# StefanHeng/ECG-Representation-Learning

Measured on AMD Instinct MI355X. Metric: 12-lead ECG records/sec pre-train step, ViT-Base bf16 @ 1/2/4/8 MI355X, higher is better.
Workload: dtype bf16

## Files before the change

### __graft_entry__.py

```python
import os
import subprocess
import sys

ROOT = os.path.dirname(os.path.abspath(__file__))
CSRC = os.path.join(ROOT, 'ecg-representation-learning_amd', 'csrc')
if ROOT not in sys.path:
    sys.path.insert(0, ROOT)


def build() -> None:
    env = dict(os.environ)
    env.setdefault('HIPCC', '/opt/rocm/bin/hipcc')
    jobs = f'-j{min(8, os.cpu_count() or 1)}'
    subprocess.run(['make', '-C', CSRC, jobs, 'all'], check=True, env=env)
    import ecg_representation_learning_amd as E
    lib = E.hip.lib()
    assert lib.ecgvit_abi_version() == E.hip.ABI_VERSION
    for name in E.hip.SIGNATURES:
        getattr(lib, name)
    r = subprocess.run(['make', '-C', CSRC, jobs, 'tools'], env=env)
    if r.returncode != 0:
        print('WARNING: the tools library did not build (the product library did); tests that need tools/toolslib.py will fail', file=sys.stderr)


def smoke() -> None:
    import torch
    import ecg_representation_learning_amd as E
    from oracle import vit_oracle as O
    assert torch.cuda.is_available(), 'smoke() needs cuda:0'
    torch.manual_seed(77)
    conf = E.EcgVitConfig(max_signal_length=1000, patch_size=20, hidden_size=128, num_hidden_layers=2,
                          num_attention_heads=2, intermediate_size=256, hidden_dropout_prob=0., attention_probs_dropout_prob=0.)
    x, y = O.synthetic_batch(4, length=1000, seed=77)
    ref = O.OracleEcgVit(config=conf)
    ref.train()
    out_ref = ref(sample_values=x, labels=y)
    out_ref.loss.backward()
    for dtype, tol in ((torch.float32, 1e-4), (torch.bfloat16, 3e-2)):
        m = E.EcgVit(config=conf, compute_dtype=dtype)
        m.load_state_dict(ref.state_dict())
        m.cuda().train()
        out = m(sample_values=x.cuda(), labels=y.cuda())
        out.loss.backward()
        rel = abs(float(out.loss) - float(out_ref.loss)) / abs(float(out_ref.loss))
        g = m.vit.mlp_head[1].weight.grad.cpu()
        g_ref = ref.vit.mlp_head[1].weight.grad
        grel = float((g - g_ref).norm() / g_ref.norm())
        print(f'smoke[{dtype}]: loss {float(out.loss):.6f} vs oracle {float(out_ref.loss):.6f} (rel {rel:.2e}); head-grad rel {grel:.2e}')
        assert rel < tol and grel < 30 * tol, (dtype, rel, grel)
        step = E.HipTrainStep(m, dict(n_step=10), sync_nonfinite=True)
        loss, _ = step.step(x.cuda(), y.cuda())
# ... 78 lines not shown
```

### ecg-representation-learning_amd/engine.py

```python
import math
from collections import OrderedDict

import os

import torch

from . import hip
from .hip import lib, run, ptr, stream, GEMM_NT, GEMM_NN, GEMM_TN
from .hip import EPI_BIAS, EPI_GELU, EPI_GELU_BWD, EPI_RESIDUAL, EPI_DROPOUT, EPI_COLSUM, EPI_GELU_GRAD_AUX, EPI_MUL_AUX

LN_EPS = 1e-5


def _align(n, a=8):
    return (n + a - 1) // a * a


def _numel(shape):
    n = 1
    for v in shape:
        n *= v
    return n


class ParamLayout:

    def __init__(self, named_shapes):
        self.entries = OrderedDict()
        off = 0
        for name, shape in named_shapes:
            n = _numel(shape)
            self.entries[name] = (off, tuple(shape), n)
            off = _align(off + n, 16)
        self.total = off

    def view(self, flat, name):
# ... 346 lines not shown
        if d > hip.ROW_MAX_D:
            raise ValueError(f'HIP LayerNorm kernels cover hidden_size <= {hip.ROW_MAX_D}')
        if h == 1:
            raise NotImplementedError('heads == 1 (vit_pytorch drops to_out) is not covered by the HIP path')
        if dtype == torch.bfloat16:
            if self.dh not in (64, 128):
                raise ValueError(f'bf16 fused attention needs head dim 64 or 128 (got {self.dh}); use dtype=torch.float32')
            if self.N > hip.ATTN_MAX_N:
                raise ValueError(f'bf16 fused attention covers <= {hip.ATTN_MAX_N} tokens (got {self.N}); use dtype=torch.float32')
            for nm, pv in (('hidden_dropout_prob', self.p_hidden), ('attention_probs_dropout_prob (the embedding dropout: reference ecg_vit.py:113)', self.p_emb)):
                if 0.0 < pv < 1.0 / 512:
                    raise ValueError(f'the bf16 path applies dropout in steps of 1/256: {nm}={pv} would round to no dropout; use 0, a value '
                                     f'>= 1/512, or compute_dtype=torch.float32 (exact p)')
        self.fp8 = bool(fp8_linear)
        if self.fp8:
            if dtype != torch.bfloat16:
                raise ValueError('fp8_linear needs the bf16 engine (compute_dtype=torch.bfloat16)')
            if d % 128 or f % 128:
                raise ValueError(f'fp8_linear needs hidden_size and intermediate_size to be multiples of 128 (got d={d}, f={f})')
        self.fp8_drop_dead_bf16 = self.fp8 and d % 256 == 0 and f % 256 == 0
        if saved_ffn_e4m3 and dtype != torch.bfloat16:
            raise ValueError('saved_ffn_e4m3 needs the bf16 engine (the f32 parity path keeps the f32 pre-activation)')
        self.aux8 = dtype == torch.bfloat16 if saved_ffn_e4m3 is None else bool(saved_ffn_e4m3)
        self.B = None
        self._alloc_key = None
        self._pool, self._pool_B = None, 0
        self.T = self.N
        self.act = None
        self.P32 = self.G32 = self.W = None
        self._ws = {}
        self.saved = None
        self.input_transform = None
        self.on_grads_ready = None
        self._tpw = 0

    def _set_width(self, width):
        if width == self.L:
            return
        if not 0 < width <= self.L_max or width % self.P:
            raise ValueError(f'a batch of {width} samples per record: must be a positive multiple of patch_size={self.P} '
                             f'and at most max_signal_length={self.L_max}')
        self.L, self.n = width, width // self.P
        self.N = self.n + 1

    def _gemm(self, *a, **kw):
        kw.setdefault('tiles_per_workgroup', self._tpw)
        hip.gemm(*a, **kw)

    def bind(self, pflat, gflat, wlow=None, wlow_t=None):
        lay = self.layout
        self.P32 = {k: lay.view(pflat, k) for k in lay.entries}
        self.G32 = {k: lay.view(gflat, k) for k in lay.entries}
        self.WT = {}
        if self.dtype == torch.bfloat16:
            assert wlow is not None and wlow.dtype == torch.bfloat16
            self.W = {k: lay.view(wlow, k) for k in lay.entries}
            if wlow_t is not None:
                for k in self.transposed_weight_names():
                    off, shape = lay.entries[k][0], lay.entries[k][1]
                    self.WT[k] = wlow_t[off:off + shape[0] * shape[1]].view(shape[1], shape[0])
        else:
            self.W = self.P32
        self.device = pflat.device
        if self.fp8:
            assert wlow_t is not None, 'fp8_linear runs the input gradients against the transposed weight shadows'
            names = self.transposed_weight_names()
# ... 177 lines not shown

    def _act_spec(self, B, masked, m, rows=None, N=None, mrows=None):
        T = self.dtype
        f32, u8 = torch.float32, torch.uint8
        if N is None:
            N = self.n if masked else self.N
        M, Mp = B * N, B * (N if masked else N - 1)
        if rows is not None:
            M, Mp = rows, rows - (0 if masked else B)
        d, f, h = self.d, self.f, self.h
        sp = OrderedDict()
        sp.update(patches=((Mp, self.CP), T), tok=((Mp, d), T), x0=((M, d), T))
        for i in range(self.Ly):
            l = dict(mean1=((M,), f32), rstd1=((M,), f32), xn1=((M, d), T), qkv=((M, 3 * d), T), attn=((M, d), T), x1=((M, d), T),
                     mean2=((M,), f32), rstd2=((M,), f32), xn2=((M, d), T), hpre=((M, f), u8 if self._aux8(M) else T), hact=((M, f), T), x2=((M, d), T))
            if T == torch.float32:
                l['probs'] = ((B * h * N * N,), T)
            else:
                l['lse'] = ((B * h * N,), f32)
            if self.fp8 and M >= 2048:
                l.update(xn1_8=((M * d,), u8), attn_8=((M * d,), u8), xn2_8=((M * d,), u8), hact_8=((M * f,), u8))
            for k, v in l.items():
                sp[f'L{i}.{k}'] = v
        sp.update(logits=((B, self.K), f32), xhat=((B, d), f32), hrstd=((B,), f32), loss_elem=((B, self.K), f32), loss_mean=((1,), f32),
                  dlogits=((B, self.K), f32))
        sp.update(dxa=((M, d), T), dxb=((M, d), T), dxn=((M, d), T), dqkv=((M, 3 * d), T), dattn=((M, d), T), dh=((M, f), T),
                  dtok=((Mp, d), T), dxm=((M, d), T))
        if T == torch.float32:
            sp.update(pd=((B * h * N * N,), T), dp=((B * h * N * N,), T))
        if T == torch.bfloat16 and not masked:
            sp.update({f'cls_{k}': ((B, d), T) for k in ('attn', 'x1', 'xn2', 'x2', 'dx', 'dy', 'dxn', 'dx1', 'dxm', 'dattn', 'dq')})
            sp.update(cls_hpre=((B, f), T), cls_hact=((B, f), T), cls_dh=((B, f), T), cls_lse=((B * h,), f32), cls_mean2=((B,), f32),
                      cls_rstd2=((B,), f32))
        l = lib()
        ws = max(l.ecgvit_layernorm_bwd_workspace(M, d), l.ecgvit_colsum_workspace(M, max(f, 3 * d)), 8 * ((M + 255) // 256) * f, 4096)
        if T == torch.bfloat16:
            for (mm, nn) in ((d, f), (f, d), (d, d), (3 * d, d), (d, self.CP)):
                ws = max(ws, hip.gemm_workspace_bytes(GEMM_TN, T, mm, nn, M))
        if masked:
            Rm = B * m if mrows is None else mrows
            sp.update(flag=((Mp,), u8), rows=((Rm, d), T), pred=((Rm, self.CP), T), target=((Rm, self.CP), T),
                      dpred=((Rm, self.CP), T), drows=((Rm, d), T), dmasked=((Mp, d), T), mloss=((1,), f32), l1part=((1024,), f32))
        sp['ws'] = ((ws,), u8)
        if self.fp8:
            sp['q8'] = ((M * max(f, 3 * d),), u8)
            sp['q8b'] = ((M * f,), u8)
        return sp

    def _ln_fwd(self, x, g, b, y, mean, rstd, rows, q8_site=None, y8=None):
        d = self.d
        if (self.fp8 and q8_site is not None and q8_site in self._f8_seen and rows >= 2048 and d % 256 == 0
                and d // 64 in (4, 8, 12, 16, 24, 32)):
            run.ecgvit_layernorm_fwd_q8(ptr(x), ptr(g), ptr(b), None if (y8 is not None and self._only8(rows)) else ptr(y), ptr(mean), ptr(rstd), rows, d, LN_EPS,
                                        ptr(y8 if y8 is not None else self.act['q8']),
                                        ptr(self.f8_scale[q8_site:q8_site + 1]), ptr(self.f8_amax[q8_site:q8_site + 1]), stream())
            return True
        run.ecgvit_layernorm_fwd(ptr(x), ptr(g), ptr(b), ptr(y), ptr(mean), ptr(rstd), rows, d, LN_EPS,
                                 hip.code(self.dtype), stream())
        return False

    def _ln_bwd(self, dy, x, g, mean, rstd, dres, dx, dg, db, rows):
        run.ecgvit_layernorm_bwd(ptr(dy), ptr(x), ptr(g), ptr(mean), ptr(rstd), ptr(dres), ptr(dx), ptr(dg), ptr(db),
                                 ptr(self.act['ws']), rows, self.d, hip.code(self.dtype), stream())

    def _ln_bwd_fused(self, dy, x, g, mean, rstd, dres, dx, dg, db, rows, dxm, dcolsum, p, seed, q8_site=None):
        d = self.d
# ... 146 lines not shown
            if (self.fp8 and self._pass_rows(B) >= 2048 and site in self._f8_seen and dh == 64 and 128 < N <= 512
                    and N * 3 * d * 2 < 2 ** 31):
                run.ecgvit_attention_bwd_q8(ptr(L['qkv']), ptr(L['attn']), ptr(a['dattn']), ptr(L['lse']), ptr(a['dqkv']), B, N, h, dh, self.scale,
                                            ph, seed, ptr(a['q8']), ptr(self.f8_scale[site:site + 1]), ptr(self.f8_amax[site:site + 1]), st)
                return True
            run.ecgvit_attention_bwd(ptr(L['qkv']), ptr(L['attn']), ptr(a['dattn']), ptr(L['lse']), ptr(a['dqkv']), B, N, h, dh, self.scale, ph,
                                     seed, hip.BF16, st)
        else:
            self._attn_bwd_f32(L, B, ph, seed)
        return False

    def _attention_cls_fwd(self, L, B, ph, seed):
        a, st = self.act, stream()
        h, dh, N = self.h, self.dh, self.T
        ntok = self.saved.get('ntok')
        if ntok is not None:
            run.ecgvit_attention_varlen_cls_fwd(ptr(L['qkv']), ptr(a['cls_attn']), ptr(a['cls_lse']), ptr(ntok), B, N, h, dh, self.scale, ph, seed,
                                                st)
        else:
            run.ecgvit_attention_cls_fwd(ptr(L['qkv']), ptr(a['cls_attn']), ptr(a['cls_lse']), B, N, h, dh, self.scale, ph, seed,
                                         hip.code(self.dtype), st)

    def _attention_cls_bwd(self, L, B, ph, seed):
        a, st = self.act, stream()
        h, dh, N = self.h, self.dh, self.T
        ntok = self.saved.get('ntok')
        if ntok is not None:
            run.ecgvit_attention_varlen_cls_bwd(ptr(L['qkv']), ptr(a['cls_attn']), ptr(a['cls_dattn']), ptr(a['cls_lse']), ptr(a['dqkv']),
                                                ptr(a['cls_dq']), ptr(ntok), B, N, h, dh, self.scale, ph, seed, st)
        else:
            run.ecgvit_attention_cls_bwd(ptr(L['qkv']), ptr(a['cls_attn']), ptr(a['cls_dattn']), ptr(a['cls_lse']), ptr(a['dqkv']), ptr(a['cls_dq']),
                                         B, N, h, dh, self.scale, ph, seed, hip.code(self.dtype), st)

    def _cls_block_fwd(self, L, X, B, ph, s0, lp):
        a, W, P = self.act, self.W, self.P32
        d, f, N = self.d, self.f, self.T
        M = B * N
        self._ln_fwd(X, P[lp + '0.norm.weight'], P[lp + '0.norm.bias'], L['xn1'], L['mean1'], L['rstd1'], M)
        wqkv = W[lp + '0.fn.to_qkv.weight']
        self._gemm(GEMM_NT, L['xn1'], wqkv, L['qkv'], M, 2 * d, d, d, d, 3 * d, b_off=d * d, c_off=d)
        self._gemm(GEMM_NT, L['xn1'], wqkv, L['qkv'], B, d, d, N * d, d, N * 3 * d)
        self._attention_cls_fwd(L, B, ph, s0 + 1)
        drop = EPI_DROPOUT if ph > 0 else 0
        self._gemm(GEMM_NT, a['cls_attn'], W[lp + '0.fn.to_out.0.weight'], a['cls_x1'], B, d, d, d, d, d, epilogue=EPI_BIAS | EPI_RESIDUAL | drop,
                   bias=P[lp + '0.fn.to_out.0.bias'], residual=X, ldr=N * d, dropout_p=ph, seed=s0 + 2, mask_row_pitch=N)
        self._ln_fwd(a['cls_x1'], P[lp + '1.norm.weight'], P[lp + '1.norm.bias'], a['cls_xn2'], a['cls_mean2'], a['cls_rstd2'], B)
        self._gemm(GEMM_NT, a['cls_xn2'], W[lp + '1.fn.net.0.weight'], a['cls_hact'], B, f, d, d, d, f,
                   epilogue=EPI_BIAS | EPI_GELU | EPI_GELU_GRAD_AUX | drop, bias=P[lp + '1.fn.net.0.bias'], aux=a['cls_hpre'], ldaux=f,
                   dropout_p=ph, seed=s0 + 3, mask_row_pitch=N)
        self._gemm(GEMM_NT, a['cls_hact'], W[lp + '1.fn.net.3.weight'], a['cls_x2'], B, d, f, f, f, d, epilogue=EPI_BIAS | EPI_RESIDUAL | drop,
                   bias=P[lp + '1.fn.net.3.bias'], residual=a['cls_x1'], ldr=d, dropout_p=ph, seed=s0 + 4, mask_row_pitch=N)
        return a['cls_x2']

    def forward(self, x, labels=None, weight=None, training=True, seed=0, want_mean=True, cls_only_last=False, lengths=None):
        return self._head_loss(self._trunk_pass(x, labels, weight, training, seed, cls_only_last, lengths), want_mean)

    def _head_loss(self, X, want_mean):
        a, sv, T = self.act, self.saved, hip.code(self.dtype)
        st = stream()
        B, d, rg, labels = sv['B'], self.d, sv['ragged'], sv['labels']
        pre = 'vit.'
        sv['head_pitch'] = 1 if (sv['cls_only_last'] or rg is not None) else self.N
        if rg is not None:
            run.ecgvit_gather_rows(ptr(X), ptr(rg.tok_off), ptr(a['cls_x2']), 1, rg.M, B, d, d, d, T, st)
            X = a['cls_x2']
        run.ecgvit_head_fwd(ptr(X), sv['head_pitch'], ptr(self.P32[pre + 'mlp_head.0.weight']), ptr(self.P32[pre + 'mlp_head.0.bias']),
                            ptr(self.P32[pre + 'mlp_head.1.weight']), ptr(self.P32[pre + 'mlp_head.1.bias']),
                            ptr(a['logits']), ptr(a['xhat']), ptr(a['hrstd']), B, d, self.K, LN_EPS, T, st)
        if labels is None:
            return a['logits'], None, None
        run.ecgvit_bce_fwd(ptr(a['logits']), ptr(labels), ptr(sv['weight']), ptr(a['loss_elem']),
                           ptr(a['loss_mean']) if want_mean else None, B * self.K, st)
        return a['logits'], a['loss_elem'], (a['loss_mean'] if want_mean else None)

    def _trunk_pass(self, x, labels, weight, training, seed, cls_only_last, lengths):
# ... 444 lines not shown
        i = self.Ly - 1
        L = a['layers'][i]
        lp = f'vit.transformer.layers.{i}.'
        s0 = seed + 100 * (i + 1)
        Xin = a['x0'] if i == 0 else a['layers'][i - 1]['x2']
        dY = dXc
        if ph > 0:
            run.ecgvit_dropout_apply_rows(ptr(dXc), ptr(a['cls_dy']), B, d, N, ph, s0 + 4, T, st)
            dY = a['cls_dy']
        self._colsum(dY, d, G[lp + '1.fn.net.3.bias'], B, d)
        if self._wants(lp + '1.fn.net.3.weight'):
            self._gemm(GEMM_TN, dY, a['cls_hact'], G[lp + '1.fn.net.3.weight'], d, f, B, d, f, f, workspace=ws)
        b = self._stage(i, 0)
        if not self._reach(b):
            return None, None
        self._gemm(GEMM_NN, dY, W[lp + '1.fn.net.3.weight'], a['cls_dh'], B, f, d, d, f, f, epilogue=EPI_MUL_AUX | EPI_COLSUM, aux=a['cls_hpre'],
                   ldaux=f, workspace=ws, colsum_out=G[lp + '1.fn.net.0.bias'])
        if self._wants(lp + '1.fn.net.0.weight'):
            self._gemm(GEMM_TN, a['cls_dh'], a['cls_xn2'], G[lp + '1.fn.net.0.weight'], f, d, B, f, d, d, workspace=ws)
        if not self._reach(b + 1):
            return None, None
        self._gemm(GEMM_NN, a['cls_dh'], W[lp + '1.fn.net.0.weight'], a['cls_dxn'], B, d, f, f, d, d)
        if not self._reach(b + 2):
            return None, None
        run.ecgvit_layernorm_bwd_fused_rowpitch(ptr(a['cls_dxn']), ptr(a['cls_x1']), ptr(P[lp + '1.norm.weight']), ptr(a['cls_mean2']),
                                                ptr(a['cls_rstd2']), ptr(dXc), ptr(a['cls_dx1']), ptr(G[lp + '1.norm.weight']),
                                                ptr(G[lp + '1.norm.bias']), ptr(ws), B, d, ptr(a['cls_dxm']), ptr(G[lp + '0.fn.to_out.0.bias']),
                                                ph, s0 + 2, N, T, st)
        dY = a['cls_dxm'] if ph > 0 else a['cls_dx1']
        if self._wants(lp + '0.fn.to_out.0.weight'):
            self._gemm(GEMM_TN, dY, a['cls_attn'], G[lp + '0.fn.to_out.0.weight'], d, d, B, d, d, d, workspace=ws)
        if not self._reach(b + 3):
            return None, None
        self._gemm(GEMM_NN, dY, W[lp + '0.fn.to_out.0.weight'], a['cls_dattn'], B, d, d, d, d, d)
        if not self._reach(b + 4):
            return None, None
        self._attention_cls_bwd(L, B, ph, s0 + 1)
        name = lp + '0.fn.to_qkv.weight'
        if self._wants(name):
            self._gemm(GEMM_TN, a['dqkv'], L['xn1'], G[name], 2 * d, d, M, 3 * d, d, d, workspace=ws, a_off=d, c_off=d * d)
            self._gemm(GEMM_TN, a['cls_dq'], L['xn1'], G[name], d, d, B, d, N * d, d, workspace=ws)
        if not self._reach(b + 5):
            return None, None
        wt = self.WT.get(name)
        if wt is not None and M >= 2048:
            self._gemm(GEMM_NT, a['dqkv'], wt, a['dxn'], M, d, 2 * d, 3 * d, 3 * d, d, a_off=d, b_off=d)
        else:
            self._gemm(GEMM_NN, a['dqkv'], W[name], a['dxn'], M, d, 2 * d, 3 * d, d, d, a_off=d, b_off=d * d)
        self._gemm(GEMM_NN, a['cls_dq'], W[name], a['dxn'], B, d, d, d, d, N * d, epilogue=hip.EPI_ACCUM)
        if not self._reach(b + 6):
            return None, None
        dres.zero_()
        run.ecgvit_scatter_rows(ptr(a['cls_dx1']), ptr(self._cls_rows(B)), ptr(dres), B, N, 1, d, d, d, T, st)
        if i > 0:
            lq = f'vit.transformer.layers.{i - 1}.'
            self._ln_bwd_fused(a['dxn'], Xin, P[lp + '0.norm.weight'], L['mean1'], L['rstd1'], dres, out, G[lp + '0.norm.weight'],
                               G[lp + '0.norm.bias'], M, a['dxm'], G[lq + '1.fn.net.3.bias'], ph, seed + 100 * i + 4)
        else:
            self._ln_bwd(a['dxn'], Xin, P[lp + '0.norm.weight'], L['mean1'], L['rstd1'], dres, out, G[lp + '0.norm.weight'], G[lp + '0.norm.bias'], M)
        self._ready(f'layer{i}')
        return out, dres

    def _cls_rows(self, B):
        t = getattr(self, '_cls_idx', None)
        if t is None or t.numel() < B or t.device != self.device:
            t = self._cls_idx = torch.zeros(max(B, 1), dtype=torch.int32, device=self.device)
        return t[:B]

    def _attn_bwd_f32(self, L, B, ph, seed):
        d, h, dh, N = self.d, self.h, self.dh, self.T
        a = self.act
        qkv, P, dqkv, dO, dP = L['qkv'], L['probs'], a['dqkv'], a['dattn'], a['dp']
        sq, so, sp = (N * 3 * d, dh), (N * d, dh), (h * N * N, N * N)
        Pd = P
        if ph > 0:
            Pd = a['pd']
            self._drop_apply_f32(P, Pd, B * h * N * N, ph, seed)
        self._gemm(GEMM_TN, Pd, dO, dqkv, N, dh, N, N, d, 3 * d, batch=(B, h), strideA=sp, strideB=so, strideC=sq, c_off=2 * d)
        self._gemm(GEMM_NT, dO, qkv, dP, N, N, dh, d, 3 * d, N, batch=(B, h), strideA=so, strideB=sq, strideC=sp, b_off=2 * d)
        if ph > 0:
# ... 61 lines not shown
```

### ecg-representation-learning_amd/hip.py

```python
import ctypes
import os
from ctypes import c_int, c_int32, c_int64, c_uint64, c_float, c_double, c_void_p, c_char_p, POINTER, Structure, byref

import torch

_PKG_DIR = os.path.dirname(os.path.abspath(__file__))
LIB_PATH = os.path.join(_PKG_DIR, 'libecgvit_hip.so')

ABI_VERSION = 6
F32, BF16, FP8_E4M3, BF8_E5M2 = 0, 1, 2, 3
GEMM_NT, GEMM_NN, GEMM_TN = 0, 1, 2
EPI_BIAS, EPI_GELU, EPI_GELU_BWD, EPI_RESIDUAL, EPI_ACCUM, EPI_DROPOUT, EPI_COLSUM = 1, 2, 4, 8, 16, 32, 64
EPI_GELU_GRAD_AUX, EPI_MUL_AUX, EPI_QUANT_OUT, EPI_NO_OUT, EPI_AUX8 = 128, 256, 512, 1024, 2048

ACC_INIT, ACC_ADD, ACC_FOLD = 0, 1, 2
KERNEL_NONE, KERNEL_GEMM_F32, KERNEL_GEMM_BF16, KERNEL_GEMM_NT, KERNEL_GEMM_WGRAD = 0, 1, 2, 3, 4
POOL_CLS, POOL_MEAN = 0, 1
ATTN_MAX_N, ROW_MAX_D = 2048, 2048
FIT_TARGETS, FIT_BINS = 16, 256
DENOISE_MAX_LEN, DENOISE_MAX_LEN_TILED = 32768, 33554432
DENOISE_MAX_TAPS = 9
DENOISE_MAX_POINTS, DENOISE_MAX_ROBUST_ITERS = 1024, 10
DENOISE_NLM_RUN, DENOISE_NLM_MAX_THREADS = 15, 512
DENOISE_LOESS_LDS = 4096
DENOISE_MAX_TILES = 65535
RESAMPLE_MAX_LEN, RESAMPLE_MAX_CHIRP = 33554432, 16777216
RESAMPLE_MAX_GENERIC, RESAMPLE_MAX_GRID_Y = 65536, 65535
TOK_MAX_CLUSTERS, TOK_MAX_LOCAL_TRIALS = 65536, 16
TOK_SEED_SPAN, TOK_DBSCAN_TILE = 1024, 256

_ERR = {1: 'ECGVIT_EINVAL (unsupported shape / argument)', 2: 'ECGVIT_ELAUNCH (HIP launch failure)'}


class HipLibraryMissing(ImportError):
    pass


class GemmDesc(Structure):
    _fields_ = [
        ('layout', c_int32), ('dtype', c_int32), ('out_dtype', c_int32), ('epilogue', c_int32),
        ('M', c_int32), ('N', c_int32), ('K', c_int32), ('batch1', c_int32), ('batch2', c_int32),
        ('A', c_void_p), ('lda', c_int64), ('strideA1', c_int64), ('strideA2', c_int64),
        ('B', c_void_p), ('ldb', c_int64), ('strideB1', c_int64), ('strideB2', c_int64),
        ('C', c_void_p), ('ldc', c_int64), ('strideC1', c_int64), ('strideC2', c_int64),
        ('bias', c_void_p), ('residual', c_void_p), ('ldr', c_int64), ('aux', c_void_p), ('ldaux', c_int64),
        ('alpha', c_float), ('dropout_p', c_float), ('dropout_seed', c_uint64),
        ('workspace', c_void_p), ('workspace_bytes', c_int64), ('colsum_out', c_void_p), ('tiles_per_workgroup', c_int32),
        ('q8_out', c_void_p), ('ldq8', c_int64), ('q8_scale', c_void_p), ('q8_amax', c_void_p), ('q8_format', c_int32),
        ('scale_a', c_void_p), ('scale_b', c_void_p),
    ]

# ... 80 lines not shown
    'ecgvit_fit_select': (c_int, [_P, _P, _I, _I, _I, _P]),
    'ecgvit_tok_assign': (c_int, [_P, _P, _L, _P, _P, _P, _L, _I, _I, _L, _I, _I, _P, _I, _P, _P, _P, _P, _P, _P]),
    'ecgvit_tok_workspace': (c_int64, [_I, _I]),
    'ecgvit_tok_update': (c_int, [_P, _P, _L, _P, _P, _P, _L, _I, _I, _L, _I, _I, _P, _P, _I, _P, _P, _I, _P]),
    'ecgvit_tok_seed_workspace': (c_int64, [_I, _L, _I, _I, _I]),
    'ecgvit_tok_seed': (c_int, [_P, _P, _L, _P, _P, _P, _L, _I, _I, _L, _I, _I, _I, _I, _L, _P, _P, _P, _P, _P, _I, _P]),
    'ecgvit_tok_decode': (c_int, [_P, _P, _L, _P, _P, _P, _L, _I, _I, _L, _I, _P, _P, _P, _I, _P]),
    'ecgvit_tok_segments': (c_int, [_P, _P, _L, _P, _P, _P, _L, _I, _I, _L, _I, _I, _P, _P, _P, _P]),
    'ecgvit_tok_dbscan_tile': (c_int, []),
    'ecgvit_tok_dbscan_rows': (c_int, [_I]),
    'ecgvit_tok_dbscan_count': (c_int, [_P, _I, _I, _F, _I, _I, _P, _P]),
    'ecgvit_tok_dbscan_link': (c_int, [_P, _I, _I, _F, _I, _I, _P, _P]),
    'ecgvit_tok_dbscan_flatten': (c_int, [_P, _I, _P, _P]),
    'ecgvit_tok_dbscan_border': (c_int, [_P, _I, _P, _P, _I, _I, _F, _I, _I, _P, _P]),
    'ecgvit_denoise_workspace': (c_int64, [_I, _I, _I]),
    'ecgvit_filtfilt': (c_int, [_P, _P, _P, _L, _P, _I, _I, _I, _I, POINTER(c_double), POINTER(c_double), POINTER(c_double), _I, _P, _P]),
    'ecgvit_nlm_sigma': (c_int, [_P, _P, _L, _P, _I, _I, _I, _P, _P, _P]),
    'ecgvit_nlm_denoise': (c_int, [_P, _P, _P, _L, _P, _I, _I, _I, _P, _D, _I, _I, _P]),
    'ecgvit_rloess': (c_int, [_P, _P, _P, _L, _P, _I, _I, _I, _I, _I, _D, _I, _I, _I, _P, _P]),
    'ecgvit_denoise_workspace_long': (c_int64, [_I, _I, _I]),
    'ecgvit_filtfilt_long': (c_int, [_P, _P, _P, _L, _P, _I, _I, _I, _I, POINTER(c_double), POINTER(c_double), POINTER(c_double), _I, _P, _P]),
    'ecgvit_nlm_sigma_long': (c_int, [_P, _P, _L, _P, _I, _I, _I, _P, _P, _P]),
    'ecgvit_nlm_denoise_tiled': (c_int, [_P, _P, _P, _L, _P, _I, _I, _I, _P, _D, _I, _I, _I, _P]),
    'ecgvit_rloess_tiled': (c_int, [_P, _P, _P, _L, _P, _I, _I, _I, _I, _I, _D, _I, _I, _I, _P, _I, _P]),
    'ecgvit_resample_plan': (c_int, [_I, POINTER(c_int), _I]),
    'ecgvit_resample_workspace': (c_int64, [_I, _I, _I, _I]),
    'ecgvit_resample': (c_int, [_P, _P, _P, _L, _P, _L, _I, _I, _I, _I, _P, _P, _P, _P]),
    'ecgvit_resample_chirp_length': (c_int, [_I]),
    'ecgvit_resample_chirp_workspace': (c_int64, [_I, _I, _I, _I, _I, _I]),
    'ecgvit_resample_chirp_filter': (c_int, [_P, _I, _I, _P, _P, _P, _P]),
    'ecgvit_resample_chirp': (c_int, [_P, _P, _P, _L, _P, _L, _I, _I, _I, _I, _P, _P, _P, _P, _P, _P, _P, _P]),
}

_lib = None


def use_library(path):
    global LIB_PATH
    if _lib is not None:
        raise RuntimeError('use_library() must come before the first ecgvit call of the process')
    if not os.path.exists(path):
        raise HipLibraryMissing(f'{path} not found')
    LIB_PATH = os.path.abspath(path)


def lib():
    global _lib
    if _lib is None:
        if not os.path.exists(LIB_PATH):
            raise HipLibraryMissing(
                f'{LIB_PATH} not found: build it with `python -c "import __graft_entry__ as g; g.build()"` '
                f'(or `make -C {os.path.join(_PKG_DIR, "csrc")}`). There is no CPU / eager fallback.')
        l = ctypes.CDLL(LIB_PATH)
        for name, (res, args) in SIGNATURES.items():
            fn = getattr(l, name)
            fn.restype, fn.argtypes = res, args
        _lib = l
    return _lib


def check(rc, what):
    if rc != 0:
        raise RuntimeError(f'{what}: {_ERR.get(rc, rc)}')


_QUERIES = frozenset(('ecgvit_abi_version', 'ecgvit_gemm_kernel', 'ecgvit_resample_plan', 'ecgvit_resample_chirp_length', 'ecgvit_tok_dbscan_tile',
                      'ecgvit_tok_dbscan_rows'))


class _Run:

    def __getattr__(self, name):
        if name not in SIGNATURES or name in _QUERIES or SIGNATURES[name][0] is not c_int:
            raise AttributeError(f'{name}: not an entry point that returns a status (queries go through lib())')
        fns = vars(lib())

        def call(*args):
            rc = fns[name](*args)
            if rc:
                raise RuntimeError(f'{name}: {_ERR.get(rc, rc)}')
        call.__name__ = name
        setattr(self, name, call)
        return call


run = _Run()


def ptr(t):
    return None if t is None else t.data_ptr()


def stream():
    return torch.cuda.current_stream().cuda_stream


def code(dtype):
    if dtype == torch.float32:
        return F32
    if dtype == torch.bfloat16:
        return BF16
    raise ValueError(f'unsupported activation dtype {dtype}')


def _need_cuda(*ts):
    for t in ts:
# ... 49 lines not shown
```

### include/ecgvit_hip.h

```cpp
#ifndef ECGVIT_HIP_H
#define ECGVIT_HIP_H

#include <stdint.h>

#ifdef __cplusplus
extern "C" {
#endif

#define ECGVIT_OK 0
#define ECGVIT_EINVAL 1
#define ECGVIT_ELAUNCH 2

#define ECGVIT_F32 0
#define ECGVIT_BF16 1
#define ECGVIT_FP8_E4M3 2
#define ECGVIT_BF8_E5M2 3

const char *ecgvit_version(void);
int ecgvit_abi_version(void);

#define ECGVIT_GEMM_NT 0
#define ECGVIT_GEMM_NN 1
#define ECGVIT_GEMM_TN 2

// ... 83 lines not shown
                               void *dxm, float *dcolsum, float dropout_p, uint64_t seed, int dtype, void *stream);

int ecgvit_layernorm_bwd_fused_rowpitch(const void *dy, const void *x, const float *gamma, const float *mean, const float *rstd,
                                        const void *dres, void *dx, float *dgamma, float *dbeta, void *partial, int64_t rows, int d,
                                        void *dxm, float *dcolsum, float dropout_p, uint64_t seed, int mask_row_pitch, int dtype, void *stream);

int ecgvit_layernorm_bwd_fused_q8(const void *dy, const void *x, const float *gamma, const float *mean, const float *rstd,
                                  const void *dres, void *dx, float *dgamma, float *dbeta, void *partial, int64_t rows, int d,
                                  void *dxm, float *dcolsum, float dropout_p, uint64_t seed, void *g8, const float *q8_scale,
                                  float *q8_amax, void *stream);

int ecgvit_dropout_apply(const void *in, void *out, int64_t count, float dropout_p, uint64_t seed, int dtype, void *stream);
int ecgvit_dropout_apply_rows(const void *in, void *out, int64_t rows, int cols, int mask_row_pitch, float dropout_p, uint64_t seed, int dtype,
                              void *stream);

int64_t ecgvit_colsum_workspace(int64_t M, int N);
int ecgvit_colsum(const void *in, int64_t ld, float *out, void *partial, int64_t M, int N, int dtype, void *stream);

#define ECGVIT_ATTN_MAX_N 2048
int ecgvit_attention_fwd(const void *qkv, void *out, float *lse, int B, int N, int h, int dh, float scale,
                         float dropout_p, uint64_t seed, int dtype, void *stream);
int ecgvit_attention_fwd_q8(const void *qkv, void *out, float *lse, int B, int N, int h, int dh, float scale, float dropout_p,
                            uint64_t seed, void *out8, const float *q8_scale, float *q8_amax, void *stream);
int ecgvit_attention_bwd(const void *qkv, const void *out, const void *dout, const float *lse, void *dqkv,
                         int B, int N, int h, int dh, float scale, float dropout_p, uint64_t seed, int dtype,
                         void *stream);
int ecgvit_attention_bwd_q8(const void *qkv, const void *out, const void *dout, const float *lse, void *dqkv,
                            int B, int N, int h, int dh, float scale, float dropout_p, uint64_t seed, void *dqkv8,
                            const float *q8_scale, float *q8_amax, void *stream);
int ecgvit_attention_cls_fwd(const void *qkv, void *out_cls, float *lse_cls, int B, int N, int h, int dh, float scale, float dropout_p,
                             uint64_t seed, int dtype, void *stream);
int ecgvit_attention_cls_bwd(const void *qkv, const void *out_cls, const void *dout_cls, const float *lse_cls, void *dqkv, void *dq_cls,
                             int B, int N, int h, int dh, float scale, float dropout_p, uint64_t seed, int dtype, void *stream);
int ecgvit_attention_probs(const void *qkv, const float *lse, float *probs, int B, int N, int h, int dh, float scale, int dtype,
                           void *stream);
int ecgvit_attention_varlen_fwd(const void *qkv, void *out, float *lse, const int32_t *n_tok, int B, int N, int h, int dh, float scale,
                                float dropout_p, uint64_t seed, void *stream);
int ecgvit_attention_varlen_bwd(const void *qkv, const void *out, const void *dout, const float *lse, void *dqkv, const int32_t *n_tok,
                                int B, int N, int h, int dh, float scale, float dropout_p, uint64_t seed, void *stream);
int ecgvit_attention_varlen_cls_fwd(const void *qkv, void *out_cls, float *lse_cls, const int32_t *n_tok, int B, int N, int h, int dh,
                                    float scale, float dropout_p, uint64_t seed, void *stream);
int ecgvit_attention_varlen_cls_bwd(const void *qkv, const void *out_cls, const void *dout_cls, const float *lse_cls, void *dqkv,
                                    void *dq_cls, const int32_t *n_tok, int B, int N, int h, int dh, float scale, float dropout_p,
                                    uint64_t seed, void *stream);
int ecgvit_attention_ragged_fwd(const void *qkv, void *out, float *lse, const int32_t *n_tok, const int32_t *tok_off, int B, int N, int h,
                                int dh, float scale, float dropout_p, uint64_t seed, void *stream);
int ecgvit_attention_ragged_bwd(const void *qkv, const void *out, const void *dout, const float *lse, void *dqkv, const int32_t *n_tok,
                                const int32_t *tok_off, int B, int N, int h, int dh, float scale, float dropout_p, uint64_t seed, void *stream);
int ecgvit_attention_ragged_cls_fwd(const void *qkv, void *out_cls, float *lse_cls, const int32_t *n_tok, const int32_t *tok_off, int B,
                                    int N, int h, int dh, float scale, float dropout_p, uint64_t seed, void *stream);
int ecgvit_attention_ragged_cls_bwd(const void *qkv, const void *out_cls, const void *dout_cls, const float *lse_cls, void *dqkv,
                                    void *dq_cls, const int32_t *n_tok, const int32_t *tok_off, int B, int N, int h, int dh, float scale,
                                    float dropout_p, uint64_t seed, void *stream);
int ecgvit_softmax_rows(float *S, int64_t rows, int N, int64_t ld, void *stream);
int ecgvit_softmax_rows_varlen(float *S, const int32_t *n_tok, int B, int h, int N, int64_t ld, void *stream);
int ecgvit_softmax_bwd_rows(const float *P, float *dP, int64_t rows, int N, int64_t ld, float scale, void *stream);

int ecgvit_head_fwd(const void *X, int N, const float *gamma, const float *beta, const float *W, const float *bias,
                    float *logits, float *xhat, float *rstd, int B, int d, int K, float eps, int dtype, void *stream);
int ecgvit_bce_fwd(const float *logits, const float *labels, const float *weight, float *loss_elem, float *loss_mean,
                   int64_t count, void *stream);
int ecgvit_bce_bwd(const float *logits, const float *labels, const float *weight, const float *gscalar,
                   const float *gelem, float gscale, float *dlogits, int64_t count, void *stream);
int ecgvit_head_bwd(const float *dlogits, const float *xhat, const float *rstd, const float *gamma, const float *beta,
                    const float *W, float *dW, float *dbias, float *dgamma, float *dbeta, void *dX, int N, int B, int d,
                    int K, int dtype, void *stream);
// ... 140 lines not shown
```

Baseline: 7350.

## Fold CLS-only last-block attention through weights instead of full K/V projections

For the final CLS-only transformer block, attention is rewritten algebraically. Instead of projecting every token to K and V, the CLS query is folded into the K weight and the attention-weighted sum is taken over normalized inputs, with the V projection applied afterwards. New HIP kernels do the per-head dot products, softmax with dropout and weighted sums, using split hi/lo bf16 MFMA to keep near-f32 accuracy, plus a matching backward that writes dxn directly. This is meant to remove the M×2d K/V projection GEMMs and their backward in that block. In exchange it adds several small kernel launches, f32 scratch buffers, and a numerical path that differs from the original.

```diff
diff --git a/__graft_entry__.py b/__graft_entry__.py
--- a/__graft_entry__.py
+++ b/__graft_entry__.py
@@ -16,7 +16,7 @@
     import ecg_representation_learning_amd as E
     lib = E.hip.lib()
     assert lib.ecgvit_abi_version() == E.hip.ABI_VERSION
-    for name in E.hip.SIGNATURES:
+    for name in list(E.hip.SIGNATURES) + list(E.hip.SIGNATURES_CLS_FOLD):
         getattr(lib, name)
     r = subprocess.run(['make', '-C', CSRC, jobs, 'tools'], env=env)
     if r.returncode != 0:
diff --git a/ecg-representation-learning_amd/csrc/attention_cls_fold.hip b/ecg-representation-learning_amd/csrc/attention_cls_fold.hip
--- /dev/null
+++ b/ecg-representation-learning_amd/csrc/attention_cls_fold.hip
@@ -0,0 +1,309 @@
+#include "common.h"
+#include "../../include/ecgvit_hip_cls_fold.h"
+
+namespace {
+
+constexpr int CF_HP = ECGVIT_CLS_FOLD_MAX_H;
+constexpr int CF_CW = ECGVIT_CLS_FOLD_COLS;
+constexpr int CF_TW = 64;
+constexpr int CF_PP = ECGVIT_CLS_FOLD_MAX_N + 8;
+constexpr int CF_XP = CF_CW + 8;
+
+__device__ __forceinline__ void cf_split(float x, bf16_t &hi, bf16_t &lo) {
+    hi = (bf16_t)x;
+    lo = (bf16_t)(x - (float)hi);
+}
+__device__ __forceinline__ f32x4 cf_mfma(bf16x8 a, bf16x8 b, f32x4 c) { return __builtin_amdgcn_mfma_f32_16x16x32_bf16(a, b, c, 0, 0, 0); }
+
+__global__ __launch_bounds__(256) void cf_dot_kernel(const bf16_t *__restrict__ xn, const float *__restrict__ v, float *__restrict__ out, int N, int h,
+                                                     int d, float alpha) {
+    extern __shared__ __attribute__((aligned(16))) unsigned char cf_smem[];
+    const int pitch = d + 8;
+    bf16_t *vh = reinterpret_cast<bf16_t *>(cf_smem), *vl = vh + CF_HP * pitch;
+    const int b = blockIdx.y;
+    const float *vb = v + (int64_t)b * h * d;
+    const int chunks = d >> 3;
+    for (int c = threadIdx.x; c < CF_HP * chunks; c += 256) {
+        const int head = c / chunks, ch = c - head * chunks;
+        bf16x8 hi, lo;
+        if (head < h) {
+            const f32x4 a0 = *reinterpret_cast<const f32x4 *>(vb + (int64_t)head * d + ch * 8);
+            const f32x4 a1 = *reinterpret_cast<const f32x4 *>(vb + (int64_t)head * d + ch * 8 + 4);
+#pragma unroll
+            for (int t = 0; t < 4; ++t) {
+                bf16_t x, y;
+                cf_split(a0[t], x, y); hi[t] = x; lo[t] = y;
+                cf_split(a1[t], x, y); hi[4 + t] = x; lo[4 + t] = y;
+            }
+        } else {
+#pragma unroll
+            for (int t = 0; t < 8; ++t) { hi[t] = (bf16_t)0.f; lo[t] = (bf16_t)0.f; }
+        }
+        *reinterpret_cast<bf16x8 *>(vh + head * pitch + ch * 8) = hi;
+        *reinterpret_cast<bf16x8 *>(vl + head * pitch + ch * 8) = lo;
+    }
+    __syncthreads();
+    const int wave = threadIdx.x >> 6, lane = threadIdx.x & 63, r = lane & 15, g = lane >> 4;
+    const int j0 = blockIdx.x * CF_TW + wave * 16;
+    if (j0 >= N) return;
+    const int row = min(j0 + r, N - 1);
+    const bf16_t *xr = xn + ((int64_t)b * N + row) * d + g * 8;
+    const bf16_t *ph = vh + r * pitch + g * 8, *pl = vl + r * pitch + g * 8;
+    f32x4 acc = {0.f, 0.f, 0.f, 0.f};
+    for (int k = 0; k < d; k += 128) {
+        bf16x8 a[4];
+#pragma unroll
+        for (int s = 0; s < 4; ++s) a[s] = *reinterpret_cast<const bf16x8 *>(xr + k + 32 * s);
+#pragma unroll
+        for (int s = 0; s < 4; ++s) {
+            acc = cf_mfma(a[s], *reinterpret_cast<const bf16x8 *>(ph + k + 32 * s), acc);
+            acc = cf_mfma(a[s], *reinterpret_cast<const bf16x8 *>(pl + k + 32 * s), acc);
+        }
+    }
+    if (r < h) {
+        float *o = out + ((int64_t)b * h + r) * N;
+#pragma unroll
+        for (int i = 0; i < 4; ++i) {
+            const int j = j0 + 4 * g + i;
+            if (j < N) o[j] = alpha * acc[i];
+        }
+    }
+}
+
+constexpr int CF_RV = ECGVIT_CLS_FOLD_MAX_N / 64;
+
+template <bool DROP>
+__global__ __launch_bounds__(256) void cf_softmax_kernel(float *p, float *__restrict__ pd, float *__restrict__ lse, int rows, int N, uint64_t seed,
+                                                         uint32_t thresh, float inv_keep) {
+    const int lane = threadIdx.x & 63;
+    const int bh = blockIdx.x * 4 + (threadIdx.x >> 6);
+    if (bh >= rows) return;
+    const float *sr = p + (int64_t)bh * N;
+    float v[CF_RV];
+    float m = -INFINITY;
+#pragma unroll
+    for (int i = 0; i < CF_RV; ++i) {
+        const int j = lane + 64 * i;
+        v[i] = j < N ? sr[j] : -INFINITY;
+        m = fmaxf(m, v[i]);
+    }
+    m = wave_max(m);
+    float sum = 0.f;
+#pragma unroll
+    for (int i = 0; i < CF_RV; ++i) sum += lane + 64 * i < N ? __expf(v[i] - m) : 0.f;
+    const float l = m + __logf(wave_sum(sum));
+    const uint32_t smix = seed_mix(seed), quad0 = (uint32_t)bh * (uint32_t)N * (uint32_t)((N + 3) >> 2);
+#pragma unroll
+    for (int i = 0; i < CF_RV; ++i) {
+        const int j = lane + 64 * i;
+        if (j < N) {
+            const float pj = __expf(v[i] - l);
+            float mult = 1.f;
+            if constexpr (DROP) {
+                const uint32_t hsh = quad_hash(smix, quad0 + (uint32_t)(j >> 2));
+                mult = ((hsh >> (8 * (j & 3))) & 0xFFu) >= thresh ? inv_keep : 0.f;
+            }
+            p[(int64_t)bh * N + j] = pj;
+            pd[(int64_t)bh * N + j] = pj * mult;
+        }
+    }
+    if (lane == 0) lse[bh] = l;
+}
+
+__global__ __launch_bounds__(256) void cf_ds_kernel(const float *__restrict__ p, const float *__restrict__ pd, float *__restrict__ dpd, int rows, int N) {
+    const int lane = threadIdx.x & 63;
+    const int bh = blockIdx.x * 4 + (threadIdx.x >> 6);
+    if (bh >= rows) return;
+    const int64_t base = (int64_t)bh * N;
+    float t[CF_RV];
+    float D = 0.f;
+#pragma unroll
+    for (int i = 0; i < CF_RV; ++i) {
+        const int j = lane + 64 * i;
+        t[i] = j < N ? pd[base + j] * dpd[base + j] : 0.f;
+        D += t[i];
+    }
+    D = wave_sum(D);
+#pragma unroll
+    for (int i = 0; i < CF_RV; ++i) {
+        const int j = lane + 64 * i;
+        if (j < N) dpd[base + j] = t[i] - p[base + j] * D;
+    }
+}
+
+__global__ __launch_bounds__(256) void cf_wsum_kernel(const bf16_t *__restrict__ xn, const float *__restrict__ t, float *__restrict__ out, int N, int h,
+                                                      int d, float alpha) {
+    __shared__ __attribute__((aligned(16))) bf16_t th[CF_HP * CF_PP];
+    __shared__ __attribute__((aligned(16))) bf16_t tl[CF_HP * CF_PP];
+    __shared__ __attribute__((aligned(16))) bf16_t xs[32 * CF_XP];
+    const int b = blockIdx.y, c0 = blockIdx.x * CF_CW;
+    const int NP = (N + 31) & ~31;
+    for (int i = threadIdx.x; i < CF_HP * NP; i += 256) {
+        const int head = i / NP, j = i - head * NP;
+        const float x = (head < h && j < N) ? t[((int64_t)b * h + head) * N + j] : 0.f;
+        bf16_t hi, lo;
+        cf_split(x, hi, lo);
+        th[head * CF_PP + j] = hi;
+        tl[head * CF_PP + j] = lo;
+    }
+    const int wave = threadIdx.x >> 6, lane = threadIdx.x & 63, r = lane & 15, g = lane >> 4;
+    const bf16_t *xb = xn + (int64_t)b * N * d + c0;
+    u32x4 st[2];
+    auto load = [&](int kt) {
+#pragma unroll
+        for (int i = 0; i < 2; ++i) {
+            const int ch = threadIdx.x + 256 * i, row = ch >> 4, cc = ch & 15, tok = kt * 32 + row;
+            st[i] = tok < N ? *reinterpret_cast<const u32x4 *>(xb + (int64_t)tok * d + cc * 8) : u32x4{0u, 0u, 0u, 0u};
+        }
+    };
+    f32x4 acc[2] = {{0.f, 0.f, 0.f, 0.f}, {0.f, 0.f, 0.f, 0.f}};
+    const int nk = NP >> 5;
+    load(0);
+    for (int kt = 0; kt < nk; ++kt) {
+        __syncthreads();
+#pragma unroll
+        for (int i = 0; i < 2; ++i) {
+            const int ch = threadIdx.x + 256 * i;
+            *reinterpret_cast<u32x4 *>(xs + (ch >> 4) * CF_XP + (ch & 15) * 8) = st[i];
+        }
+        __syncthreads();
+        if (kt + 1 < nk) load(kt + 1);
+        const bf16x8 ah = *reinterpret_cast<const bf16x8 *>(th + r * CF_PP + kt * 32 + g * 8);
+        const bf16x8 al = *reinterpret_cast<const bf16x8 *>(tl + r * CF_PP + kt * 32 + g * 8);
+#pragma unroll
+        for (int ct = 0; ct < 2; ++ct) {
+            const int col = (wave * 2 + ct) * 16 + r;
+            bf16x8 bf;
+#pragma unroll
+            for (int e = 0; e < 8; ++e) bf[e] = xs[(8 * g + e) * CF_XP + col];
+            acc[ct] = cf_mfma(ah, bf, acc[ct]);
+            acc[ct] = cf_mfma(al, bf, acc[ct]);
+        }
+    }
+#pragma unroll
+    for (int ct = 0; ct < 2; ++ct)
+#pragma unroll
+        for (int i = 0; i < 4; ++i) {
+            const int head = 4 * g + i;
+            if (head < h) out[((int64_t)b * h + head) * d + c0 + (wave * 2 + ct) * 16 + r] = alpha * acc[ct][i];
+        }
+}
+
+__global__ __launch_bounds__(256) void cf_dxn_kernel(const float *__restrict__ ds, const float *__restrict__ pd, const float *__restrict__ u,
+                                                     const float *__restrict__ w, bf16_t *__restrict__ dxn, int N, int h, int d, float scale) {
+    __shared__ __attribute__((aligned(16))) bf16_t os[4][16 * CF_XP];
+    constexpr int CT = CF_CW / 16;
+    const int b = blockIdx.y, c0 = blockIdx.x * CF_CW;
+    const int wave = threadIdx.x >> 6, lane = threadIdx.x & 63, r = lane & 15, g = lane >> 4;
+    const int hb = 8 * (g & 1);
+    const float *vsrc = (g < 2 ? u : w) + (int64_t)b * h * d + c0 + r;
+    bf16x8 bh[CT], bl[CT];
+#pragma unroll
+    for (int ct = 0; ct < CT; ++ct)
+#pragma unroll
+        for (int e = 0; e < 8; ++e) {
+            const float x = hb + e < h ? vsrc[(int64_t)(hb + e) * d + ct * 16] : 0.f;
+            bf16_t hi, lo;
+            cf_split(x, hi, lo);
+            bh[ct][e] = hi; bl[ct][e] = lo;
+        }
+    const float *src = (g < 2 ? ds : pd) + (int64_t)b * h * N;
+    const float mul = g < 2 ? scale : 1.f;
+    for (int t0 = 0; t0 < N; t0 += CF_TW) {
+        const int j0 = t0 + wave * 16;
+        const bool live = j0 < N;
+        if (live) {
+            const int j = min(j0 + r, N - 1);
+            bf16x8 ah, al;
+#pragma unroll
+            for (int e = 0; e < 8; ++e) {
+                const float x = hb + e < h ? mul * src[(int64_t)(hb + e) * N + j] : 0.f;
+                bf16_t hi, lo;
+                cf_split(x, hi, lo);
+                ah[e] = hi; al[e] = lo;
+            }
+#pragma unroll
+            for (int ct = 0; ct < CT; ++ct) {
+                f32x4 acc = {0.f, 0.f, 0.f, 0.f};
+                acc = cf_mfma(al, bh[ct], acc);
+                acc = cf_mfma(ah, bl[ct], acc);
+                acc = cf_mfma(ah, bh[ct], acc);
+#pragma unroll
+                for (int i = 0; i < 4; ++i) os[wave][(4 * g + i) * CF_XP + ct * 16 + r] = (bf16_t)acc[i];
+            }
+        }
+        __syncthreads();
+        if (live) {
+#pragma unroll
+            for (int i = 0; i < 4; ++i) {
+                const int ch = lane + 64 * i, row = ch >> 4, cc = ch & 15;
+                if (j0 + row < N)
+                    *reinterpret_cast<u32x4 *>(dxn + ((int64_t)b * N + j0 + row) * d + c0 + cc * 8) =
+                        *reinterpret_cast<const u32x4 *>(&os[wave][row * CF_XP + cc * 8]);
+            }
+        }
+        __syncthreads();
+    }
+}
+
+bool cf_al16(const void *p) { return reinterpret_cast<uintptr_t>(p) % 16 == 0; }
+
+bool cf_args_ok(int B, int N, int h, int d) {
+    return B >= 1 && B <= 65535 && N >= 1 && N <= ECGVIT_CLS_FOLD_MAX_N && h >= 1 && h <= ECGVIT_CLS_FOLD_MAX_H && d >= ECGVIT_CLS_FOLD_COLS &&
+           d <= ECGVIT_CLS_FOLD_MAX_D && d % ECGVIT_CLS_FOLD_COLS == 0;
+}
+
+int cf_dot(const bf16_t *xn, const float *v, float *out, int B, int N, int h, int d, float alpha, hipStream_t s) {
+    const size_t lds = (size_t)2 * CF_HP * (d + 8) * sizeof(bf16_t);
+    hipLaunchKernelGGL(cf_dot_kernel, dim3((unsigned)((N + CF_TW - 1) / CF_TW), (unsigned)B), dim3(256), lds, s, xn, v, out, N, h, d, alpha);
+    ECGVIT_CHECK_LAUNCH();
+    return ECGVIT_OK;
+}
+
+int cf_wsum(const bf16_t *xn, const float *t, float *out, int B, int N, int h, int d, float alpha, hipStream_t s) {
+    hipLaunchKernelGGL(cf_wsum_kernel, dim3((unsigned)(d / CF_CW), (unsigned)B), dim3(256), 0, s, xn, t, out, N, h, d, alpha);
+    ECGVIT_CHECK_LAUNCH();
+    return ECGVIT_OK;
+}
+
+}
+
+extern "C" {
+
+int ecgvit_attention_cls_fold_fwd(const void *xn, const float *u, float *z, float *p, float *p_drop, float *lse, int B, int N, int h, int d, float scale,
+                                  float dropout_p, uint64_t seed, void *stream) {
+    if (!xn || !u || !z || !p || !p_drop || !lse || !cf_args_ok(B, N, h, d) || !cf_al16(xn) || !cf_al16(u)) return ECGVIT_EINVAL;
+    if (dropout_p < 0.f || dropout_p >= 1.f || (dropout_p > 0.f && dropout_threshold8(dropout_p) == 0)) return ECGVIT_EINVAL;
+    const hipStream_t s = as_stream(stream);
+    const bf16_t *x = (const bf16_t *)xn;
+    const uint32_t th = dropout_threshold8(dropout_p);
+    const float ik = dropout_inv_keep8(dropout_p);
+    int rc = cf_dot(x, u, p, B, N, h, d, scale, s);
+    if (rc != ECGVIT_OK) return rc;
+    const int rows = B * h;
+    const dim3 grid((unsigned)((rows + 3) / 4));
+    if (th) hipLaunchKernelGGL(cf_softmax_kernel<true>, grid, dim3(256), 0, s, p, p_drop, lse, rows, N, seed, th, ik);
+    else hipLaunchKernelGGL(cf_softmax_kernel<false>, grid, dim3(256), 0, s, p, p_drop, lse, rows, N, seed, th, ik);
+    ECGVIT_CHECK_LAUNCH();
+    return cf_wsum(x, p_drop, z, B, N, h, d, 1.f, s);
+}
+
+int ecgvit_attention_cls_fold_bwd(const void *xn, const float *u, const float *w, const float *p, const float *p_drop, float *ws, float *r, void *dxn,
+                                  int B, int N, int h, int d, float scale, void *stream) {
+    if (!xn || !u || !w || !p || !p_drop || !ws || !r || !dxn || !cf_args_ok(B, N, h, d) || !cf_al16(xn) || !cf_al16(w) || !cf_al16(dxn))
+        return ECGVIT_EINVAL;
+    const hipStream_t s = as_stream(stream);
+    const bf16_t *x = (const bf16_t *)xn;
+    int rc = cf_dot(x, w, ws, B, N, h, d, 1.f, s);
+    if (rc != ECGVIT_OK) return rc;
+    const int rows = B * h;
+    hipLaunchKernelGGL(cf_ds_kernel, dim3((unsigned)((rows + 3) / 4)), dim3(256), 0, s, p, p_drop, ws, rows, N);
+    ECGVIT_CHECK_LAUNCH();
+    rc = cf_wsum(x, ws, r, B, N, h, d, scale, s);
+    if (rc != ECGVIT_OK) return rc;
+    hipLaunchKernelGGL(cf_dxn_kernel, dim3((unsigned)(d / CF_CW), (unsigned)B), dim3(256), 0, s, ws, p_drop, u, w, (bf16_t *)dxn, N, h, d, scale);
+    ECGVIT_CHECK_LAUNCH();
+    return ECGVIT_OK;
+}
+
+}
diff --git a/ecg-representation-learning_amd/engine.py b/ecg-representation-learning_amd/engine.py
--- a/ecg-representation-learning_amd/engine.py
+++ b/ecg-representation-learning_amd/engine.py
@@ -2,6 +2,7 @@
 from collections import OrderedDict
 
 import os
+import weakref
 
 import torch
 
@@ -414,6 +415,7 @@
         self.saved = None
         self.input_transform = None
         self.on_grads_ready = None
+        self._cls_zeroed = {}
         self._tpw = 0
 
     def _set_width(self, width):
@@ -657,6 +659,11 @@
             sp.update({f'cls_{k}': ((B, d), T) for k in ('attn', 'x1', 'xn2', 'x2', 'dx', 'dy', 'dxn', 'dx1', 'dxm', 'dattn', 'dq')})
             sp.update(cls_hpre=((B, f), T), cls_hact=((B, f), T), cls_dh=((B, f), T), cls_lse=((B * h,), f32), cls_mean2=((B,), f32),
                       cls_rstd2=((B,), f32))
+            if self._cls_fold_ok(N):
+                R = B * h
+                sp.update(cls_q=((B, d), T), cls_qx=((R, d), T), cls_dox=((R, d), T), cls_z16=((R, d), T), cls_r16=((R, d), T), cls_y=((R, d), T))
+                sp.update({f'cls_{k}': ((R, d), f32) for k in ('u', 'w', 'z', 'r')})
+                sp.update({f'cls_{k}': ((R * N,), f32) for k in ('p', 'pd', 'fws')})
         l = lib()
         ws = max(l.ecgvit_layernorm_bwd_workspace(M, d), l.ecgvit_colsum_workspace(M, max(f, 3 * d)), 8 * ((M + 255) // 256) * f, 4096)
         if T == torch.bfloat16:
@@ -869,15 +876,73 @@
             run.ecgvit_attention_cls_bwd(ptr(L['qkv']), ptr(a['cls_attn']), ptr(a['cls_dattn']), ptr(a['cls_lse']), ptr(a['dqkv']), ptr(a['cls_dq']),
                                          B, N, h, dh, self.scale, ph, seed, hip.code(self.dtype), st)
 
+    def _cls_fold_ok(self, N):
+        return (self.dtype == torch.bfloat16 and not self.fp8 and self.dh == 64 and self.h * self.dh == self.d and N <= hip.CLS_FOLD_MAX_N
+                and self.h <= hip.CLS_FOLD_MAX_H and self.d % hip.CLS_FOLD_COLS == 0 and self.d <= hip.CLS_FOLD_MAX_D)
+
+    def _cls_fold_heads(self, B, name=None):
+        t = getattr(self, '_cls_hidx', None)
+        if t is None or t.shape[0] < B or t.device != self.device:
+            t = self._cls_hidx = (torch.arange(self.h, dtype=torch.int32, device=self.device) * (self.h + 1)).repeat(max(B, 1), 1).contiguous()
+        if name is not None:
+            slab, seen = self._pool[name], self._cls_zeroed.get(name)
+            if seen is None or seen() is not slab:
+                slab.zero_()
+                self._cls_zeroed[name] = weakref.ref(slab)
+        return t[:B]
+
+    def _cls_fold_fwd(self, L, B, ph, seed, wqkv, name):
+        a, st, T = self.act, stream(), hip.code(self.dtype)
+        d, h, dh, N = self.d, self.h, self.dh, self.T
+        R = B * h
+        idx = self._cls_fold_heads(B, 'cls_qx')
+        self._gemm(GEMM_NT, L['xn1'], wqkv, a['cls_q'], B, d, d, N * d, d, d)
+        run.ecgvit_scatter_rows(ptr(a['cls_q']), ptr(idx), ptr(a['cls_qx']), B, h * h, h, dh, dh, dh, T, st)
+        self._cls_fold_in(a['cls_qx'], name, a['cls_u'], R, 1)
+        run.ecgvit_attention_cls_fold_fwd(ptr(L['xn1']), ptr(a['cls_u']), ptr(a['cls_z']), ptr(a['cls_p']), ptr(a['cls_pd']), ptr(a['cls_lse']), B, N,
+                                          h, d, self.scale, ph, seed, st)
+        run.ecgvit_cast_f32_to_bf16(ptr(a['cls_z']), ptr(a['cls_z16']), R * d, st)
+        self._gemm(GEMM_NT, a['cls_z16'], wqkv, a['cls_y'], R, d, d, d, d, d, b_off=2 * d * d)
+        run.ecgvit_gather_rows(ptr(a['cls_y']), ptr(idx), ptr(a['cls_attn']), B, h * h, h, dh, dh, dh, T, st)
+
+    def _cls_fold_in(self, X, name, out, R, part):
+        d = self.d
+        wt = self.WT.get(name)
+        if wt is not None and R >= 2048:
+            self._gemm(GEMM_NT, X, wt, out, R, d, d, d, 3 * d, d, b_off=part * d)
+        else:
+            self._gemm(GEMM_NN, X, self.W[name], out, R, d, d, d, d, d, b_off=part * d * d)
+
+    def _cls_fold_bwd(self, L, B, name, b):
+        a, st, T = self.act, stream(), hip.code(self.dtype)
+        d, h, dh, N = self.d, self.h, self.dh, self.T
+        R = B * h
+        idx = self._cls_fold_heads(B, 'cls_dox')
+        run.ecgvit_scatter_rows(ptr(a['cls_dattn']), ptr(idx), ptr(a['cls_dox']), B, h * h, h, dh, dh, dh, T, st)
+        self._cls_fold_in(a['cls_dox'], name, a['cls_w'], R, 2)
+        run.ecgvit_attention_cls_fold_bwd(ptr(L['xn1']), ptr(a['cls_u']), ptr(a['cls_w']), ptr(a['cls_p']), ptr(a['cls_pd']), ptr(a['cls_fws']),
+                                          ptr(a['cls_r']), ptr(a['dxn']), B, N, h, d, self.scale, st)
+        run.ecgvit_cast_f32_to_bf16(ptr(a['cls_r']), ptr(a['cls_r16']), R * d, st)
+        if self._wants(name):
+            self._gemm(GEMM_TN, a['cls_qx'], a['cls_r16'], self.G32[name], d, d, R, d, d, d, workspace=a['ws'], c_off=d * d)
+            self._gemm(GEMM_TN, a['cls_dox'], a['cls_z16'], self.G32[name], d, d, R, d, d, d, workspace=a['ws'], c_off=2 * d * d)
+        if self._wants(name) or self._reach(b + 5):
+            self._gemm(GEMM_NT, a['cls_r16'], self.W[name], a['cls_y'], R, d, d, d, d, d, b_off=d * d)
+            run.ecgvit_gather_rows(ptr(a['cls_y']), ptr(idx), ptr(a['cls_dq']), B, h * h, h, dh, dh, dh, T, st)
+
     def _cls_block_fwd(self, L, X, B, ph, s0, lp):
         a, W, P = self.act, self.W, self.P32
         d, f, N = self.d, self.f, self.T
         M = B * N
         self._ln_fwd(X, P[lp + '0.norm.weight'], P[lp + '0.norm.bias'], L['xn1'], L['mean1'], L['rstd1'], M)
         wqkv = W[lp + '0.fn.to_qkv.weight']
-        self._gemm(GEMM_NT, L['xn1'], wqkv, L['qkv'], M, 2 * d, d, d, d, 3 * d, b_off=d * d, c_off=d)
-        self._gemm(GEMM_NT, L['xn1'], wqkv, L['qkv'], B, d, d, N * d, d, N * 3 * d)
-        self._attention_cls_fwd(L, B, ph, s0 + 1)
+        self.saved['cls_fold'] = self.saved.get('ntok') is None and self._cls_fold_ok(N)
+        if self.saved['cls_fold']:
+            self._cls_fold_fwd(L, B, ph, s0 + 1, wqkv, lp + '0.fn.to_qkv.weight')
+        else:
+            self._gemm(GEMM_NT, L['xn1'], wqkv, L['qkv'], M, 2 * d, d, d, d, 3 * d, b_off=d * d, c_off=d)
+            self._gemm(GEMM_NT, L['xn1'], wqkv, L['qkv'], B, d, d, N * d, d, N * 3 * d)
+            self._attention_cls_fwd(L, B, ph, s0 + 1)
         drop = EPI_DROPOUT if ph > 0 else 0
         self._gemm(GEMM_NT, a['cls_attn'], W[lp + '0.fn.to_out.0.weight'], a['cls_x1'], B, d, d, d, d, d, epilogue=EPI_BIAS | EPI_RESIDUAL | drop,
                    bias=P[lp + '0.fn.to_out.0.bias'], residual=X, ldr=N * d, dropout_p=ph, seed=s0 + 2, mask_row_pitch=N)
@@ -1388,20 +1453,25 @@
             self._gemm(GEMM_TN, dY, a['cls_attn'], G[lp + '0.fn.to_out.0.weight'], d, d, B, d, d, d, workspace=ws)
         if not self._reach(b + 3):
             return None, None
+        fold = self.saved['cls_fold']
         self._gemm(GEMM_NN, dY, W[lp + '0.fn.to_out.0.weight'], a['cls_dattn'], B, d, d, d, d, d)
         if not self._reach(b + 4):
             return None, None
-        self._attention_cls_bwd(L, B, ph, s0 + 1)
         name = lp + '0.fn.to_qkv.weight'
+        if fold:
+            self._cls_fold_bwd(L, B, name, b)
+        else:
+            self._attention_cls_bwd(L, B, ph, s0 + 1)
         if self._wants(name):
-            self._gemm(GEMM_TN, a['dqkv'], L['xn1'], G[name], 2 * d, d, M, 3 * d, d, d, workspace=ws, a_off=d, c_off=d * d)
+            if not fold:
+                self._gemm(GEMM_TN, a['dqkv'], L['xn1'], G[name], 2 * d, d, M, 3 * d, d, d, workspace=ws, a_off=d, c_off=d * d)
             self._gemm(GEMM_TN, a['cls_dq'], L['xn1'], G[name], d, d, B, d, N * d, d, workspace=ws)
         if not self._reach(b + 5):
             return None, None
         wt = self.WT.get(name)
-        if wt is not None and M >= 2048:
+        if not fold and wt is not None and M >= 2048:
             self._gemm(GEMM_NT, a['dqkv'], wt, a['dxn'], M, d, 2 * d, 3 * d, 3 * d, d, a_off=d, b_off=d)
-        else:
+        elif not fold:
             self._gemm(GEMM_NN, a['dqkv'], W[name], a['dxn'], M, d, 2 * d, 3 * d, d, d, a_off=d, b_off=d * d)
         self._gemm(GEMM_NN, a['cls_dq'], W[name], a['dxn'], B, d, d, d, d, N * d, epilogue=hip.EPI_ACCUM)
         if not self._reach(b + 6):
diff --git a/ecg-representation-learning_amd/hip.py b/ecg-representation-learning_amd/hip.py
--- a/ecg-representation-learning_amd/hip.py
+++ b/ecg-representation-learning_amd/hip.py
@@ -17,6 +17,7 @@
 KERNEL_NONE, KERNEL_GEMM_F32, KERNEL_GEMM_BF16, KERNEL_GEMM_NT, KERNEL_GEMM_WGRAD = 0, 1, 2, 3, 4
 POOL_CLS, POOL_MEAN = 0, 1
 ATTN_MAX_N, ROW_MAX_D = 2048, 2048
+CLS_FOLD_MAX_N, CLS_FOLD_MAX_H, CLS_FOLD_MAX_D, CLS_FOLD_COLS = 512, 16, 896, 128
 FIT_TARGETS, FIT_BINS = 16, 256
 DENOISE_MAX_LEN, DENOISE_MAX_LEN_TILED = 32768, 33554432
 DENOISE_MAX_TAPS = 9
@@ -163,6 +164,11 @@
     'ecgvit_resample_chirp': (c_int, [_P, _P, _P, _L, _P, _L, _I, _I, _I, _I, _P, _P, _P, _P, _P, _P, _P, _P]),
 }
 
+SIGNATURES_CLS_FOLD = {
+    'ecgvit_attention_cls_fold_fwd': (c_int, [_P, _P, _P, _P, _P, _P, _I, _I, _I, _I, _F, _F, _U, _P]),
+    'ecgvit_attention_cls_fold_bwd': (c_int, [_P, _P, _P, _P, _P, _P, _P, _P, _I, _I, _I, _I, _F, _P]),
+}
+
 _lib = None
 
 
@@ -183,7 +189,7 @@
                 f'{LIB_PATH} not found: build it with `python -c "import __graft_entry__ as g; g.build()"` '
                 f'(or `make -C {os.path.join(_PKG_DIR, "csrc")}`). There is no CPU / eager fallback.')
         l = ctypes.CDLL(LIB_PATH)
-        for name, (res, args) in SIGNATURES.items():
+        for name, (res, args) in list(SIGNATURES.items()) + list(SIGNATURES_CLS_FOLD.items()):
             fn = getattr(l, name)
             fn.restype, fn.argtypes = res, args
         _lib = l
@@ -202,7 +208,8 @@
 class _Run:
 
     def __getattr__(self, name):
-        if name not in SIGNATURES or name in _QUERIES or SIGNATURES[name][0] is not c_int:
+        sig = SIGNATURES.get(name) or SIGNATURES_CLS_FOLD.get(name)
+        if sig is None or name in _QUERIES or sig[0] is not c_int:
             raise AttributeError(f'{name}: not an entry point that returns a status (queries go through lib())')
         fns = vars(lib())
 
diff --git a/include/ecgvit_hip.h b/include/ecgvit_hip.h
--- a/include/ecgvit_hip.h
+++ b/include/ecgvit_hip.h
@@ -139,6 +139,10 @@
                              uint64_t seed, int dtype, void *stream);
 int ecgvit_attention_cls_bwd(const void *qkv, const void *out_cls, const void *dout_cls, const float *lse_cls, void *dqkv, void *dq_cls,
                              int B, int N, int h, int dh, float scale, float dropout_p, uint64_t seed, int dtype, void *stream);
+#define ECGVIT_CLS_FOLD_MAX_N 512
+#define ECGVIT_CLS_FOLD_MAX_H 16
+#define ECGVIT_CLS_FOLD_MAX_D 896
+#define ECGVIT_CLS_FOLD_COLS 128
 int ecgvit_attention_probs(const void *qkv, const float *lse, float *probs, int B, int N, int h, int dh, float scale, int dtype,
                            void *stream);
 int ecgvit_attention_varlen_fwd(const void *qkv, void *out, float *lse, const int32_t *n_tok, int B, int N, int h, int dh, float scale,
diff --git a/include/ecgvit_hip_cls_fold.h b/include/ecgvit_hip_cls_fold.h
--- /dev/null
+++ b/include/ecgvit_hip_cls_fold.h
@@ -0,0 +1,19 @@
+#ifndef ECGVIT_HIP_CLS_FOLD_H
+#define ECGVIT_HIP_CLS_FOLD_H
+
+#include "ecgvit_hip.h"
+
+#ifdef __cplusplus
+extern "C" {
+#endif
+
+int ecgvit_attention_cls_fold_fwd(const void *xn, const float *u, float *z, float *p, float *p_drop, float *lse, int B, int N, int h, int d,
+                                  float scale, float dropout_p, uint64_t seed, void *stream);
+int ecgvit_attention_cls_fold_bwd(const void *xn, const float *u, const float *w, const float *p, const float *p_drop, float *ws, float *r,
+                                  void *dxn, int B, int N, int h, int d, float scale, void *stream);
+
+#ifdef __cplusplus
+}
+#endif
+
+#endif
```

Result: no change. 7393, median of 6 (+0.6%).
